# ChalmersPhotonicsLab/QAMpy

Hardware: AMD Instinct MI355X
Metric: equalised MSym/s (2-pol, 2 SPS) (higher is better)
Workload: dtype f32

## Files before the change

qampy_amd/csrc/api.hip:

```cpp
#include "common.h"
#include <stdlib.h>
#include <atomic>
#include <mutex>
#include <vector>
#include <unordered_map>
#include <string.h>

namespace qh {

thread_local hipStream_t g_stream = nullptr;
static thread_local hipStream_t g_streams[4] = {nullptr, nullptr, nullptr, nullptr};
int g_device = -1;
static thread_local std::string g_err;
static std::mutex g_mu;

void set_error(const std::string &s) { g_err = s; }

int hip_fail(hipError_t e, const char *what, const char *file, int line)
{
    g_err = std::string(hipGetErrorString(e)) + " in " + what + " (" + file + ":" + std::to_string(line) + ")";
    (void)hipGetLastError();
    return QH_ERR_HIP;
}

// ... 33 lines not shown
    }
    int n = 0;
    if (hipGetDeviceCount(&n) != hipSuccess || n <= 0) {
        (void)hipGetLastError();
        set_error("no HIP device visible: libqampy_hip needs a gfx950 (MI355X) GPU, there is no CPU fallback");
        return QH_ERR_NODEVICE;
    }
    if (device < 0 || device >= n) { set_error("device index out of range"); return QH_ERR_ARG; }
    hipDeviceProp_t prop;
    QH_HIP(hipGetDeviceProperties(&prop, device));
    if (strncmp(prop.gcnArchName, "gfx950", 6) != 0) {
        set_error(std::string("device is ") + prop.gcnArchName + ", libqampy_hip is built for gfx950 only");
        return QH_ERR_NODEVICE;
    }
    QH_HIP(hipSetDevice(device));
    int prio_least = 0, prio_greatest = 0;
    QH_HIP(hipDeviceGetStreamPriorityRange(&prio_least, &prio_greatest));
    for (int i = 0; i < 4; i++) {
        if (g_streams[i]) { (void)hipStreamDestroy(g_streams[i]); g_streams[i] = nullptr; }
        if (i == 2) {
            const int reserved = reserved_cus();
            const int ncu = prop.multiProcessorCount;
            if (reserved > 0 && reserved < ncu) {
                std::vector<uint32_t> mask((ncu + 31) / 32, 0u);
                for (int c = reserved; c < ncu; c++) mask[c / 32] |= 1u << (c % 32);
                if (hipExtStreamCreateWithCUMask(&g_streams[i], (uint32_t)mask.size(), mask.data()) == hipSuccess) continue;
                (void)hipGetLastError();
                g_streams[i] = nullptr;
            }
        }
        QH_HIP(hipStreamCreateWithPriority(&g_streams[i], hipStreamNonBlocking, i == 2 ? prio_least : prio_greatest));
    }
    g_stream = g_streams[0];
    g_device = device;
    return QH_OK;
}

hipStream_t side_stream() { return g_stream == g_streams[0] ? g_streams[1] : g_streams[0]; }
hipStream_t helper_stream() { return g_streams[3]; }

int ensure_init()
{
    if (g_stream) return QH_OK;
    return init_device(g_device >= 0 ? g_device : 0);
}

thread_local void *g_scratch[SCRATCH_SLOTS] = {nullptr};
thread_local size_t g_scratch_n[SCRATCH_SLOTS] = {0};
thread_local unsigned g_scratch_epoch = 0;
static std::atomic<int> g_form[FORM_COUNT];
struct FormName { const char *key, *env; };
static const FormName FORM_NAMES[FORM_COUNT] = {
    {"trainer", "QAMPY_HIP_TRAINER"}, {"pit_form", "QAMPY_HIP_PIT_FORM"}, {"seg_lanes", "QAMPY_HIP_SEG_LANES"}, {"pit_probe", "QAMPY_HIP_PIT_PROBE"},
    {"bps", "QAMPY_HIP_BPS"}};
static int form_parse(int k, const char *v, int *out)
{
    if (!v || !v[0]) { *out = 0; return 0; }
    switch (k) {
    case FORM_TRAINER: *out = v[0] == 'd' ? 1 : (v[0] == 'l' ? 2 : (v[0] == 'i' ? 3 : (v[0] == 'a' || v[0] == '0' ? 0 : -1))); break;
    case FORM_PIT: *out = v[0] == 's' ? 1 : (v[0] == 'b' ? 2 : (v[0] == 'a' || v[0] == '0' ? 0 : -1)); break;
    case FORM_SEG_LANES: { const int n = atoi(v); *out = (n == 8 || n == 16 || n == 0) ? n : -1; break; }
    case FORM_BPS: *out = v[0] == 't' ? 1 : (v[0] == 'l' ? 2 : (v[0] == 'a' || v[0] == '0' ? 0 : -1)); break;
    default: *out = atoi(v) != 0 ? 1 : 0; break;
    }
    return *out < 0 ? -1 : 0;
}
static const int g_form_env_read = [] {
    for (int k = 0; k < FORM_COUNT; k++) {
        int v = 0;
        if (form_parse(k, getenv(FORM_NAMES[k].env), &v) == 0) g_form[k].store(v);
    }
    return 0;
}();
int form(FormKey k) { return g_form[k].load(std::memory_order_relaxed); }
const char *trainer_force()
{
    switch (form(FORM_TRAINER)) {
    case 1: return "direct";
    case 2: return "lookahead";
    case 3: return "iterative";
    default: return "";
    }
}
static constexpr int POOL_CLASSES = 48, POOL_KEEP = 8;
static constexpr size_t POOL_BYTES = (size_t)24 << 30;
static std::vector<void *> g_pool[POOL_CLASSES];
static size_t g_pool_bytes = 0;
static void pool_release();
static int pool_class(size_t bytes) { int k = 8; while (((size_t)1 << k) < bytes && k < POOL_CLASSES - 1) k++; return k; }
int pool_alloc(size_t bytes, void **p, size_t *cap)
{
    const int k = pool_class(bytes);
    *cap = (size_t)1 << k;
    {
        std::lock_guard<std::mutex> lk(g_mu);
        if (!g_pool[k].empty()) { *p = g_pool[k].back(); g_pool[k].pop_back(); g_pool_bytes -= *cap; return QH_OK; }
    }
    hipError_t e = hipMalloc(p, *cap);
    if (e == hipErrorOutOfMemory) {
        (void)hipGetLastError();
        (void)hipDeviceSynchronize();
        pool_release();
        e = hipMalloc(p, *cap);
    }
    QH_HIP(e);
    return QH_OK;
}
// ... 348 lines not shown
```

qampy_amd/csrc/common.h:

```cpp
#pragma once
#include <hip/hip_runtime.h>
#include <stdint.h>
#include <string>
#include "../../include/qampy_hip.h"

namespace qh {

extern thread_local hipStream_t g_stream;
extern int g_device;
void set_error(const std::string &s);
int hip_fail(hipError_t e, const char *what, const char *file, int line);

#define QH_HIP(call)                                                        \
    do {                                                                    \
        hipError_t _e = (call);                                             \
        if (_e != hipSuccess) return qh::hip_fail(_e, #call, __FILE__, __LINE__); \
    } while (0)

#define QH_REQUIRE(cond, msg)                                   \
    do {                                                        \
        if (!(cond)) { qh::set_error(msg); return QH_ERR_ARG; } \
    } while (0)

#define QH_WAVE_FIRST() __builtin_amdgcn_s_setprio(3)

int ensure_init();
hipStream_t side_stream();
hipStream_t helper_stream();
enum FormKey { FORM_TRAINER = 0, FORM_PIT, FORM_SEG_LANES, FORM_PIT_PROBE, FORM_BPS, FORM_COUNT };
int form(FormKey k);
const char *trainer_force();
double gram_budget_gb();
int pit_timing_mode();
int default_tier();
double default_tier_tol();
constexpr int SCRATCH_SLOTS = 22;
constexpr int SCRATCH_TWOSTAGE = 16;
constexpr int SCRATCH_FOE = 17;
constexpr int SCRATCH_IMPAIR = 18;
constexpr int SCRATCH_PMD = 19;
constexpr int SCRATCH_TXRESP = 20;
constexpr int SCRATCH_SOS = 21;
int scratch(int slot, size_t bytes, void **p);
unsigned scratch_epoch();

int bps_twostage_recover_f32(const void *E, int nm, int64_t L, const void *angles, int A, int B, const void *symbols, int M, int N, int32_t *idx1,
                             int32_t *idx2, void *ph, void *Eout);
int bps_twostage_recover_f64(const void *E, int nm, int64_t L, const void *angles, int A, int B, const void *symbols, int M, int N, int32_t *idx1,
                             int32_t *idx2, void *ph, void *Eout);

int pool_alloc(size_t bytes, void **p, size_t *cap);
void pool_free(void *p, size_t cap);

struct DevBuf {
    void *p = nullptr;
    size_t n = 0, cap = 0;
    ~DevBuf() { if (p) pool_free(p, cap); }
    int alloc(size_t bytes) {
        n = bytes;
        return pool_alloc(bytes ? bytes : 1, &p, &cap);
    }
    int from_host(const void *h, size_t bytes) {
        int rc = alloc(bytes);
        if (rc) return rc;
        if (bytes) QH_HIP(hipMemcpyAsync(p, h, bytes, hipMemcpyHostToDevice, g_stream));
        return QH_OK;
    }
    int to_host(void *h, size_t bytes) const {
        if (bytes) QH_HIP(hipMemcpyAsync(h, p, bytes, hipMemcpyDeviceToHost, g_stream));
        return QH_OK;
    }
};

template <typename R> struct Cx { R re, im; };

template <typename R> struct Cx2T;
template <> struct Cx2T<float> { using type = float2; };
template <> struct Cx2T<double> { using type = double2; };

template <typename R> __device__ __forceinline__ Cx<R> ldg(const Cx<R> *p)
{
    using V = typename Cx2T<R>::type;
// ... 82 lines not shown
```

qampy_amd/csrc/train_pit.h:

```cpp
#pragma once
#include <atomic>
#include <chrono>
#include <vector>
#include "train_impl.h"
#include "train_seg.h"

namespace qh {

typedef qh_pit_report PitCtrl;

constexpr double PIT_CONTRACT = 0.2;
constexpr int PIT_PROBE = 128;
constexpr int PIT_SEEDWIN = 512;
constexpr int PIT_MAXSEG = 65536;

__host__ __device__ inline int pit_symmetry(int method)
{
    switch (method) {
    case QH_M_CMA: case QH_M_SGNCMA: case QH_M_RDE: return 0;
    case QH_M_CMA2: return 2;
    default: return 4;
    }
}

// ... 1220 lines not shown
            const int k = k0 + 4 * i;
            if (k < np) {
                Zf a = abuf[i];
                abuf[i] = lda(k + 4 * PF);
                if (MODE == 0) a.y = -a.y;
                const Zf b = bp[(size_t)k * PIT_MBP];
                rr = __builtin_amdgcn_mfma_f32_16x16x4f32(a.x, b.x, rr, 0, 0, 0);
                ii = __builtin_amdgcn_mfma_f32_16x16x4f32(a.y, b.y, ii, 0, 0, 0);
                im = __builtin_amdgcn_mfma_f32_16x16x4f32(a.x, b.y, im, 0, 0, 0);
                im = __builtin_amdgcn_mfma_f32_16x16x4f32(a.y, b.x, im, 0, 0, 0);
            }
        }
    }
    const int cl = lane & 15;
    if (MODE == 0) {
        const int col = col0 + cl;
#pragma unroll
        for (int q = 0; q < 4; q++) {
            const int m = 16 * wave + 4 * (lane >> 4) + q;
            if (m < n && col < ncol) Out[(size_t)m * ncol + col] = Zf{rr[q] - ii[q], im[q]};
        }
    } else {
#pragma unroll
        for (int q = 0; q < 4; q++) {
            const int m = 16 * wave + 4 * (lane >> 4) + q;
            Ct[cl * (PIT_EIGMAX + 1) + m] = Zf{rr[q] - ii[q], im[q]};
        }
        __syncthreads();
        for (int cb = 0; cb < PIT_MC; cb += NCW * nw) {
#pragma unroll
            for (int q = 0; q < NCW; q++) {
                const int cc = cb + wave + nw * q, col = col0 + cc;
                if (cc < PIT_MC && col < ncol) {
                    const int s = col / fz.nsel, j = col - s * fz.nsel;
                    const size_t base = (size_t)s * wset + (size_t)fz.modes_dev[j] * n;
                    const double qr = pre ? th[q][0] : fz.theta[2 * (size_t)col], qi = pre ? th[q][1] : fz.theta[2 * (size_t)col + 1];
#pragma unroll
                    for (int h = 0; h < 2; h++) {
                        const int m = lane + 64 * h;
                        if (m < n) {
                            const Cx<R> x = pre ? xv[q][h] : fz.X[base + m];
                            const Zf d = Ct[cc * (PIT_EIGMAX + 1) + m];
                            const Cx<R> w{(R)(qr * x.re - qi * x.im + fz.damp * d.x), (R)(qr * x.im + qi * x.re + fz.damp * d.y)};
                            fz.X[base + m] = w;
                            fz.Y[base + m] = w;
                        }
                    }
                }
            }
        }
    }
}

static __global__ void __launch_bounds__(256) pit_bound_kernel(const Zf *Xe, const Zf *Ye, const Zf *Yprev, const double *lam, int n, int S, int nsel, int sym,
                                                              const PitCtrl *c, double *dfc, double *pw, double *gph, float4 *ualpha = nullptr)
{
    QH_WAVE_FIRST();
    if (c->done) return;
    const int lane = threadIdx.x & 63, bi = blockIdx.x * 4 + (threadIdx.x >> 6);
    const int nb = (S - 1) * nsel, ncol = S * nsel;
    if (bi >= nb + nsel) return;
    const bool result_probe = bi >= nb;
    const int j = result_probe ? bi - nb : bi % nsel;
    const int sb = result_probe ? S - 1 : bi / nsel;
    const Zf *pa = result_probe ? (c->passes == 0 ? Xe + (size_t)(S - 1) * nsel + j : Yprev + j) : Xe + (size_t)(sb + 1) * nsel + j;
    const size_t sa = (result_probe && c->passes != 0) ? (size_t)nsel : (size_t)ncol;
    const Zf *pb = Ye + (size_t)sb * nsel + j;
    Zf av[(PIT_EIGMAX + 63) / 64], bv[(PIT_EIGMAX + 63) / 64];
    float lv[(PIT_EIGMAX + 63) / 64];
    double A = 0, B = 0, Cr = 0, Ci = 0;
#pragma unroll
    for (int q = 0; q < (PIT_EIGMAX + 63) / 64; q++) {
        const int k = lane + 64 * q;
        av[q] = Zf{0.f, 0.f}; bv[q] = Zf{0.f, 0.f}; lv[q] = 0.f;
        if (k < n) {
            av[q] = pa[(size_t)k * sa]; bv[q] = pb[(size_t)k * ncol];
            const float l = (float)lam[k];
            lv[q] = l > 0.f ? l : 0.f;
        }
        A += (double)lv[q] * ((double)av[q].x * av[q].x + (double)av[q].y * av[q].y);
        B += (double)lv[q] * ((double)bv[q].x * bv[q].x + (double)bv[q].y * bv[q].y);
        Cr += (double)lv[q] * ((double)bv[q].x * av[q].x + (double)bv[q].y * av[q].y);
        Ci += (double)lv[q] * ((double)bv[q].y * av[q].x - (double)bv[q].x * av[q].y);
    }
    for (int o = 32; o > 0; o >>= 1) { A += __shfl_xor(A, o); B += __shfl_xor(B, o); Cr += __shfl_xor(Cr, o); Ci += __shfl_xor(Ci, o); }
    double gr = 1, gi = 0;
    if (sym == 0) {
        const double pr = sqrt(Cr * Cr + Ci * Ci);
        if (pr > 0) { gr = Cr / pr; gi = Ci / pr; }
    } else if (sym == 4 || sym == 2 || sym == 1) {
        if (sym == 4 && fabs(Ci) > fabs(Cr)) { gr = 0; gi = Ci >= 0 ? 1 : -1; }
        else if (sym == 1) gr = 1;
        else gr = Cr >= 0 ? 1 : -1;
    } else {
        const double step = 6.283185307179586 / sym;
        const double kk = rint(atan2(Ci, Cr) / step) * step;
        gr = cos(kk); gi = sin(kk);
    }
    double d2 = 0;
    const float grf = (float)gr, gif = (float)gi;
#pragma unroll
    for (int q = 0; q < (PIT_EIGMAX + 63) / 64; q++) {
        const float dr = bv[q].x - (grf * av[q].x - gif * av[q].y), di = bv[q].y - (grf * av[q].y + gif * av[q].x);
        d2 += (double)lv[q] * ((double)dr * dr + (double)di * di);
    }
    for (int o = 32; o > 0; o >>= 1) d2 += __shfl_xor(d2, o);
    if (ualpha && !result_probe) {
        float nn = 0.f, ar = 0.f, ai = 0.f;
#pragma unroll
        for (int q = 0; q < (PIT_EIGMAX + 63) / 64; q++) {
            const float dr = bv[q].x - (grf * av[q].x - gif * av[q].y), di = bv[q].y - (grf * av[q].y + gif * av[q].x);
            const float ur = lv[q] * bv[q].x, ui = lv[q] * bv[q].y;
            nn += ur * ur + ui * ui;
            ar += ur * dr + ui * di;
            ai += ur * di - ui * dr;
        }
        for (int o = 32; o > 0; o >>= 1) { nn += __shfl_xor(nn, o); ar += __shfl_xor(ar, o); ai += __shfl_xor(ai, o); }
        const float inv = nn > 0.f ? rsqrtf(nn) : 0.f;
        if (lane == 0) ualpha[bi] = float4{ar * inv, ai * inv, inv, 0.f};
    }
    if (lane == 0) {
        if (!result_probe) { gph[2 * (size_t)bi] = gr; gph[2 * (size_t)bi + 1] = gi; pw[bi] = B; }
        dfc[bi] = (A == A && B == B) ? sqrt(d2 / (B > 1e-300 ? B : 1e-300)) : 1e30;
    }
}

constexpr int PIT_RT = 1024;
template <typename R>
__global__ void __launch_bounds__(PIT_RT) pit_recur_eig_kernel(Zf *Xe, const Zf *Ye, Zf *D, const double *theta, const double *lam, int nsel, int S, int64_t T, const R *mu,
                                                               double beta, const PitCtrl *c, const float *Msum = nullptr, float damp = 1.f,
                                                               const float4 *ualpha = nullptr, const float2 *uq = nullptr)
{
    QH_WAVE_FIRST();
    if (c->done) return;
    __shared__ float4 aff[2 * PIT_RT];
    const int k = blockIdx.x, j = blockIdx.y;
    const int ncol = S * nsel;
    Zf *row = D + (size_t)k * ncol + j, *xr = Xe + (size_t)k * ncol + j;
    const Zf *yr = Ye + (size_t)k * ncol + j;
    double a = (double)*mu * c->gain * (double)T * lam[k];
    if (a < 0) a = 0;
    const float coef = c->corr_on ? (float)exp(-a * (1 + beta * a)) : 0.f;
    const float gl = (float)(c->gain * lam[k] > 0 ? c->gain * lam[k] : 0.0), betaf = (float)beta;
    const bool corr = c->corr_on != 0;
    auto cf = [&](int s) -> float {
        if (!Msum) return coef;
        const float as = gl * Msum[(size_t)s * nsel + j];
        return corr ? __expf(-as * (1.f + betaf * as)) : 0.f;
    };
    const int len = (S + PIT_RT - 1) / PIT_RT;
    const int s0 = threadIdx.x * len, s1 = s0 + len < S ? s0 + len : S;
    auto th = [&](int s) { return Zf{(float)theta[2 * ((size_t)s * nsel + j)], (float)theta[2 * ((size_t)s * nsel + j) + 1]}; };
    auto scan_op = [](float4 e, float4 l) { return float4{l.x * e.x, l.x * e.y + l.y, l.x * e.z + l.z, 0.f}; };
    if (len <= 4) {
        Zf y[4], x[4], t[5], r[4];
        t[0] = s0 > 0 && s0 < S ? th(s0 - 1) : Zf{1.f, 0.f};
#pragma unroll
        for (int q = 0; q < 4; q++) {
            const int s = s0 + q;
            const bool ok = s < s1;
            y[q] = (ok && s > 0) ? yr[(size_t)(s - 1) * nsel] : Zf{0.f, 0.f};
            x[q] = ok ? xr[(size_t)s * nsel] : Zf{0.f, 0.f};
            t[q + 1] = ok ? th(s) : Zf{1.f, 0.f};
        }
        Zf run{0.f, 0.f};
        float cq[4], clen = 1.f;
        float4 ua[4];
        float2 qq[4];
        const float lk = (float)(lam[k] > 0 ? lam[k] : 0.0);
#pragma unroll
        for (int q = 0; q < 4; q++) {
            const int s = s0 + q;
            cq[q] = (s < s1 && s > 0) ? cf(s - 1) : (s < s1 ? 0.f : 1.f);
            ua[q] = (ualpha && s < s1 && s > 0) ? ualpha[(size_t)(s - 1) * nsel + j] : float4{0.f, 0.f, 0.f, 0.f};
            qq[q] = (uq && s < s1 && s > 0) ? uq[(size_t)s * nsel + j] : float2{0.f, 0.f};
        }
        Zf uk[4];
#pragma unroll
        for (int q = 0; q < 4; q++) {
            const int s = s0 + q;
// ... 153 lines not shown
    const int s0 = threadIdx.x * len, s1 = s0 + len < n ? s0 + len : n;
    auto seg_map = [&](int s, double &A, double &B) {
        const double rho = (double)rS[s], d = (double)rE[s] - rho;
        double kappa = 0;
        if (newton && pass >= 2) {
            const double rp = (double)rPrev[s], dp = (double)dPrev[s];
            if (fabs(rho - rp) > 1e-6 * rho && fabs(d) > 1e-30) kappa = -((d - dp) / d) / ((rho - rp) / rho);
            kappa = kappa == kappa ? (kappa < 0 ? 0 : (kappa > 4 ? 4 : kappa)) : 0;
        }
        A = 1.0 - kappa * d / rho;
        B = d * (1.0 + kappa);
    };
    double Ac = 1, Bc = 0;
    for (int s = s0; s < s1; s++) { double A, B; seg_map(s, A, B); Bc = A * Bc + B; Ac = A * Ac; }
    auto comp = [](double2 e, double2 l) { return double2{l.x * e.x, l.x * e.y + l.y}; };
    const double2 pre = block_scan_excl<double2, decltype(comp), 1024>(double2{Ac, Bc}, comp, double2{1.0, 0.0}, buf);
    double run = pre.x * (double)rS[0] + pre.y;
    float worst = 0.f;
    for (int s = s0; s < s1; s++) {
        double A, B;
        seg_map(s, A, B);
        const float old = (float)rS[s];
        rPrev[s] = old; dPrev[s] = (float)((double)rE[s] - (double)old);
        if (s > 0) {
            const float nw = pass == 0 ? (float)run : old + relax * ((float)run - old);
            const float rel = fabsf(nw - old) / (fabsf(old) > 1e-30f ? fabsf(old) : 1e-30f);
            worst = (rel > worst || !(rel == rel)) ? (rel == rel ? rel : 3.0e38f) : worst;
            rS[s] = (R)nw;
            eS[s] = eE[s - 1];
        }
        run = A * run + B;
    }
    for (int o = 32; o > 0; o >>= 1) { const float w2 = __shfl_xor(worst, o); worst = worst > w2 ? worst : w2; }
    if ((threadIdx.x & 63) == 0) red[threadIdx.x >> 6] = worst;
    __syncthreads();
    if (threadIdx.x == 0) { float m = 0.f; for (int w = 0; w < 16; w++) m = m > red[w] ? m : red[w]; chg[0] = m; }
}
template <typename R> __global__ void pit_adapt_finish_kernel(R *mu, const R *rE, int n) { *mu = (R)1 / rE[n - 1]; }

struct PitInit { void *z[3]; unsigned zn[3]; void *cd[2]; const void *cs[2]; unsigned cn[2]; int64_t *modes_dev; int64_t modes[16]; int nsel; };
static __global__ void __launch_bounds__(256) pit_init_kernel(PitInit a)
{
    QH_WAVE_FIRST();
    const unsigned t = blockIdx.x * 256 + threadIdx.x, nt = gridDim.x * 256;
#pragma unroll
    for (int r = 0; r < 3; r++)
        if (a.z[r]) for (unsigned i = t; i < a.zn[r] / 4; i += nt) reinterpret_cast<uint32_t *>(a.z[r])[i] = 0u;
#pragma unroll
    for (int r = 0; r < 2; r++)
        if (a.cd[r]) for (unsigned i = t; i < a.cn[r] / 8; i += nt) reinterpret_cast<uint64_t *>(a.cd[r])[i] = reinterpret_cast<const uint64_t *>(a.cs[r])[i];
    if ((int)t < a.nsel) a.modes_dev[t] = a.modes[t];
}
constexpr int PIT_GT_THREADS = 1024;
template <typename R>
__global__ void __launch_bounds__(PIT_GT_THREADS) pit_gauge_kernel(const double *gph, int S, int nsel, PitCtrl *c, double *theta, const double *pw, int nb, int method, const Cx<R> *sy0,
                                                                   int want_corr, const PitModel *model = nullptr, const float4 *ualpha = nullptr, float2 *uq = nullptr,
                                                                   const R *mu = nullptr, int64_t T = 0, const float *Msum = nullptr)
{
    QH_WAVE_FIRST();
    if (c->done) return;
    constexpr int NT = PIT_GT_THREADS;
    __shared__ double redp[NT / 64];
    __shared__ double2 gbuf[NT / 64];
    __shared__ float4 abuf[NT / 64];
    if (gridDim.x > 1 && blockIdx.x == 1 && !(model && uq)) return;
    if (model && uq && (gridDim.x == 1 || blockIdx.x == 1)) {
        const bool corr = c->passes == 0 ? true : c->corr_on != 0;
        const int len = (S + NT - 1) / NT;
        const int s0 = threadIdx.x * len, s1 = s0 + len < S ? s0 + len : S;
        const float muT = mu ? (float)((double)*mu * (double)T) : 0.f;
        auto op = [](float4 e, float4 l) { return float4{l.x * e.x, l.x * e.y + l.y, l.z * e.z, l.z * e.w + l.w}; };
        for (int j = 0; j < nsel; j++) {
            const PitModel m = model[j];
            const bool on = corr && m.ok;
            auto cf = [&](int s, float &c1, float &c2) {
                const float t = Msum ? Msum[(size_t)s * nsel + j] : muT;
                c1 = on ? __expf(-fmaxf(m.k1, 0.f) * t) : 0.f; c2 = on ? __expf(-fmaxf(m.k2, 0.f) * t) : 0.f;
            };
            float4 loc{1.f, 0.f, 1.f, 0.f};
            for (int s = s0; s < s1; s++) {
                float b1 = 0.f, b2 = 0.f, c1 = 0.f, c2 = 0.f;
                if (s > 0) { const float4 al = ualpha[(size_t)(s - 1) * nsel + j]; b1 = m.q11 * al.x + m.q21 * al.y; b2 = m.q12 * al.x + m.q22 * al.y; cf(s - 1, c1, c2); }
                loc = op(loc, float4{c1, b1, c2, b2});
            }
            const float4 pre = block_scan_excl<float4, decltype(op), NT>(loc, op, float4{1.f, 0.f, 1.f, 0.f}, abuf);
            float r1 = pre.y, r2 = pre.w;
            for (int s = s0; s < s1; s++) {
                float b1 = 0.f, b2 = 0.f, c1 = 0.f, c2 = 0.f;
                if (s > 0) { const float4 al = ualpha[(size_t)(s - 1) * nsel + j]; b1 = m.q11 * al.x + m.q21 * al.y; b2 = m.q12 * al.x + m.q22 * al.y; cf(s - 1, c1, c2); }
                r1 = c1 * r1 + b1; r2 = c2 * r2 + b2;
                uq[(size_t)s * nsel + j] = float2{m.q11 * r1 + m.q12 * r2, m.q21 * r1 + m.q22 * r2};
            }
        }
        if (gridDim.x > 1) return;
    }
    if (c->passes == 0) {
        double ps = 0;
        for (int i = threadIdx.x; i < nb; i += NT) ps += pw[i];
        for (int o = 32; o > 0; o >>= 1) ps += __shfl_xor(ps, o);
        if ((threadIdx.x & 63) == 0) redp[threadIdx.x >> 6] = ps;
        __syncthreads();
        if (threadIdx.x == 0) {
            double tot = 0;
            for (int w = 0; w < NT / 64; w++) tot += redp[w];
            const double Py = tot / (nb > 0 ? nb : 1);
            double g = pit_gain<R>(method, Py, sy0[0]);
            if (model) {
                double gs = 0; int ng = 0;
                for (int j = 0; j < nsel; j++) if (model[j].ok) { gs += (double)model[j].g; ng++; }
                if (ng == nsel && gs > 0) g = gs / ng;
            }
            c->out_power = Py; c->gain = g;
            c->corr_on = (want_corr && g > 0 && g == g) ? 1 : 0;
        }
        __syncthreads();
    }
    const int len = (S + NT - 1) / NT;
    const int s0 = threadIdx.x * len, s1 = s0 + len < S ? s0 + len : S;
    auto cm = [](double2 x, double2 y) { return double2{x.x * y.x - x.y * y.y, x.x * y.y + x.y * y.x}; };
    const double2 *g2 = reinterpret_cast<const double2 *>(gph);
    double2 *th2 = reinterpret_cast<double2 *>(theta);
    if (len <= 4 && nsel <= 2) {
        double2 g[2][4];
#pragma unroll
        for (int j = 0; j < 2; j++)
#pragma unroll
            for (int q = 0; q < 4; q++) {
                const int s = s0 + q;
                g[j][q] = (j < nsel && s < s1 && s > 0) ? g2[(size_t)(s - 1) * nsel + j] : double2{1.0, 0.0};
            }
#pragma unroll
        for (int j = 0; j < 2; j++) {
            if (j >= nsel) break;
            const double2 prod = cm(cm(g[j][0], g[j][1]), cm(g[j][2], g[j][3]));
            double2 run = block_scan_excl<double2, decltype(cm), NT>(prod, cm, double2{1.0, 0.0}, gbuf);
#pragma unroll
            for (int q = 0; q < 4; q++) {
                const int s = s0 + q;
                run = cm(run, g[j][q]);
                if (s < s1) {
                    const double r = rsqrt(run.x * run.x + run.y * run.y);
                    th2[(size_t)s * nsel + j] = double2{run.x * r, run.y * r};
                }
            }
        }
        return;
    }
    for (int j = 0; j < nsel; j++) {
        double2 prod{1.0, 0.0};
        for (int s = s0; s < s1; s++)
            if (s > 0) prod = cm(prod, g2[(size_t)(s - 1) * nsel + j]);
        double2 run = block_scan_excl<double2, decltype(cm), NT>(prod, cm, double2{1.0, 0.0}, gbuf);
        for (int s = s0; s < s1; s++) {
            if (s > 0) run = cm(run, g2[(size_t)(s - 1) * nsel + j]);
            const double r = rsqrt(run.x * run.x + run.y * run.y);
            th2[(size_t)s * nsel + j] = double2{run.x * r, run.y * r};
        }
    }
}
template <typename R>
__global__ void __launch_bounds__(256) pit_devest_kernel(const Zf *D, const double *lam, int n, int ncol, const PitCtrl *c, float *devmax, unsigned *ticket, PitDecideArgs<R> da)
{
    QH_WAVE_FIRST();
    if (c->done) return;
    __shared__ float part[2][4][64], red[64], reds[64], redt[64], redm[64];
    const int cl = threadIdx.x & 63, kg = threadIdx.x >> 6;
    const int col = blockIdx.x * 64 + cl;
    float acc = 0.f, tap = 0.f;
    if (col < ncol) {
#pragma unroll 8
        for (int k = kg; k < n; k += 4) {
            const Zf v = D[(size_t)k * ncol + col];
            const float l = (float)lam[k], m2 = v.x * v.x + v.y * v.y;
            acc += (l > 0.f ? l : 0.f) * m2;
            tap += m2;
        }
    }
    part[0][kg][cl] = acc; part[1][kg][cl] = tap;
    __syncthreads();
    if (kg == 0) {
        acc = (part[0][0][cl] + part[0][1][cl]) + (part[0][2][cl] + part[0][3][cl]);
        tap = (part[1][0][cl] + part[1][1][cl]) + (part[1][2][cl] + part[1][3][cl]);
        red[cl] = (acc == acc) ? acc : 3.0e38f;
        reds[cl] = (acc == acc) ? acc : 3.0e38f;
        redt[cl] = (tap == tap) ? tap : 3.0e38f;
        redm[cl] = (tap == tap) ? tap : 3.0e38f;
    }
    __syncthreads();
    for (int s = 32; s > 0; s >>= 1) {
        if (threadIdx.x < s) {
            red[threadIdx.x] = red[threadIdx.x] > red[threadIdx.x + s] ? red[threadIdx.x] : red[threadIdx.x + s];
            reds[threadIdx.x] += reds[threadIdx.x + s];
            redt[threadIdx.x] += redt[threadIdx.x + s];
            redm[threadIdx.x] = redm[threadIdx.x] > redm[threadIdx.x + s] ? redm[threadIdx.x] : redm[threadIdx.x + s];
        }
        __syncthreads();
    }
    if (threadIdx.x == 0) {
        devmax[4 * blockIdx.x] = red[0]; devmax[4 * blockIdx.x + 1] = reds[0]; devmax[4 * blockIdx.x + 2] = redt[0]; devmax[4 * blockIdx.x + 3] = redm[0];
    }
    __shared__ int last;
    if (threadIdx.x == 0) {
        __threadfence();
        const unsigned t = atomicAdd(ticket, 1u);
        last = t == gridDim.x - 1;
        if (last) { *ticket = 0; __threadfence(); }
    }
    __syncthreads();
    if (!last) return;
    pit_decide_body<R>(da);
}
// ... 332 lines not shown
        if (t > seg_want) seg_want = t;
    }
    if (S == 0 && adaptive) S = (int)((TrSyms - head) / seg_want < PIT_MAXSEG ? (TrSyms - head) / seg_want : PIT_MAXSEG);
    if (S == 0) {
        R mu_h = (R)o.mu_hint;
        if (!(o.mu_hint > 0)) {
            QH_HIP(hipMemcpyAsync(&mu_h, mu_dev, sizeof(R), hipMemcpyDeviceToHost, g_stream));
            QH_HIP(hipStreamSynchronize(g_stream));
        }
        S = pit_auto_segments(TrSyms, (double)mu_h, nsel, o.acquire);
    }
    PitPlan pl = pit_plan(o, TrSyms, head, S, adaptive, o.acquire ? o.acq_chunk : 0);
    const PitSeg &sg = pl.sg;
    if (zero_err) QH_HIP(hipMemsetAsync(err, 0, (size_t)nmodes * TrSyms * Niter * sizeof(Cx<R>), g_stream));
    const int64_t npow = L < 4096 ? L : 4096;
    hipLaunchKernelGGL((pit_setup_kernel<R>), dim3(1), dim3(256), 0, g_stream, (const Cx<R> *)E, nmodes, L, npow, ntot, (const R *)mu_dev, pl.gear, pl.bound, tol, sg, ctrl, mu_acq);
    QH_HIP(hipGetLastError());
    if (TrSyms == 0 || Niter == 0) return QH_OK;
    if (sg.S < 2) {
        const double zero = 0;
        QH_HIP(hipMemcpyAsync(&ctrl->defect[0], &zero, sizeof(double), hipMemcpyHostToDevice, g_stream));
        return exact_form(ctrl, adaptive ? 1 : 0, 0, gram, 1);
    }

    TrainerForm f;
    if ((rc = trainer_form<R>(f, FORM_PASSES, method, adaptive, nmodes, ntaps, os, sg.len, (int64_t)sg.S * nsel, symbols, nsy, modes, nsel))) return rc;
    if (adaptive && !f.seg) return exact_form(ctrl, 1, 0, nullptr, 0);
    const bool decision = method == QH_M_SBD || method == QH_M_MDDMA || method == QH_M_DD;
    const bool seg_form = f.seg, use_bi = f.use_bi, block_form = f.block, pair_tab = f.pair_tab;
    const bool split = o.exchange != nullptr;
    const int own_first = split ? o.seg_first : 0, own_count = split ? o.seg_count : sg.S;
    const bool xchg_async = split && o.exchange_on_stream != 0;
    if (split) {
        QH_REQUIRE(seg_form, "train_equaliser: a capture split over processes needs the throughput form of the passes (>= 512 chains, supported tap layout)");
        QH_REQUIRE(own_first >= 0 && own_count >= 0 && own_first + own_count <= sg.S, "train_equaliser: owned segments outside the segment grid");
        QH_REQUIRE(Niter == 1, "train_equaliser: a capture split over processes is trained in one sweep");
    }

    const size_t wset = (size_t)nmodes * ntot;
    const size_t wbytes = wset * sizeof(Cx<R>);
    void *wbuf = nullptr;
    const size_t nsj = (size_t)sg.S * nsel;
    const size_t bytes_w = ((2 * (size_t)sg.S + 2) * wbytes + 63) / 64 * 64;
    if ((rc = scratch(2, bytes_w + 10 * nsj * sizeof(double) + (size_t)nsel * sizeof(int64_t) + 320 + nsj * 16 + 4 * ((nsj + 63) / 64) * sizeof(float) + 64, &wbuf))) return rc;
    Cx<R> *X = (Cx<R> *)wbuf, *Y = X + (size_t)sg.S * wset, *w_start = Y + (size_t)sg.S * wset, *w_call = w_start + wset;
    double *z = (double *)((char *)wbuf + bytes_w), *rot = z + 2 * nsj, *dfc = rot + 2 * nsj, *pw = dfc + nsj, *gph = pw + nsj, *theta = gph + 2 * nsj;
    int64_t *modes_dev = (int64_t *)(theta + 2 * nsj);
    double *uw_phi = (double *)(modes_dev + ((nsel + 7) / 8 * 8));
    int *uw_jump = (int *)(uw_phi + (size_t)sg.S * nsel);
    float *devmax = (float *)(uw_jump + (size_t)sg.S * nsel);
    const int ndev = (int)((nsj + 63) / 64);
    unsigned *ticket = (unsigned *)(devmax + 4 * (size_t)ndev);
    PitInit init{};
    init.z[0] = ticket; init.zn[0] = sizeof(unsigned);
    R *ad_rS = nullptr, *ad_rE = nullptr;
    Cx<R> *ad_eS = nullptr, *ad_eE = nullptr, *ad_errh = nullptr;
    float *ad_M = nullptr, *ad_chg = nullptr, *ad_rP = nullptr, *ad_dP = nullptr;
    if (!adaptive && head > 0) {
        void *ab = nullptr;
        if ((rc = scratch(13, (size_t)nmodes * head * sizeof(Cx<R>) + 64, &ab))) return rc;
        ad_errh = (Cx<R> *)ab;
    }
    if (adaptive) {
        void *ab = nullptr;
        const size_t nS = ((size_t)sg.S + 15) / 16 * 16;
        if ((rc = scratch(13, nS * (2 * sizeof(R) + 2 * sizeof(Cx<R>) + 3 * sizeof(float)) + 64 + (size_t)nmodes * head * sizeof(Cx<R>), &ab))) return rc;
        ad_eS = (Cx<R> *)ab; ad_eE = ad_eS + nS; ad_errh = ad_eE + nS;
        ad_rS = (R *)(ad_errh + (size_t)nmodes * head); ad_rE = ad_rS + nS;
        ad_M = (float *)(ad_rE + nS); ad_rP = ad_M + nS; ad_dP = ad_rP + nS; ad_chg = ad_dP + nS;
    }
    init.modes_dev = modes_dev; init.nsel = nsel;
    for (int j = 0; j < 16; j++) init.modes[j] = j < nsel ? modes[j] : 0;
    const bool prepared = o.prepared != nullptr && o.acquire && !adaptive && head == 0 && Niter >= 1;
    const bool need_mu = adaptive || !(o.mu_hint > 0), need_acq = o.acquire && !(o.acq_chunk > 0) && !prepared;
    R mu_acq_h = 0;
    if (need_acq) QH_HIP(hipMemcpyAsync(&mu_acq_h, mu_acq, sizeof(R), hipMemcpyDeviceToHost, g_stream));
    R mu_host = need_mu ? (R)1 : (R)o.mu_hint;
    if (need_mu) QH_HIP(hipMemcpyAsync(&mu_host, mu_dev, sizeof(R), hipMemcpyDeviceToHost, g_stream));
    if (need_mu || need_acq) QH_HIP(hipStreamSynchronize(g_stream));
    if (!adaptive && !(mu_host != 0))
        return exact_form(ctrl, 0, 0, gram, 0);
    if (o.acquire && !(o.acq_chunk > 0)) pl.acquisition(o, TrSyms, pit_acq_chunk(mu_acq_h));

    const int64_t amax = pl.amax;
    void *G = const_cast<void *>(gram);
    if (prepared) QH_REQUIRE(seg_form && o.acq_chunk > 0, "train_equaliser: a prepared acquisition belongs to throughput-form passes with acq_chunk given (qh_pit_prepare_*_dev said so)");
    if (block_form && !G && (!seg_form || amax > 0) && !prepared) {
        const int64_t n = seg_form ? pl.ngram : TrSyms;
        rc = pair_tab ? gram_build<R>(E, nmodes, L, os, ntaps, n, &G) : gram_cur_build<R>(E, nmodes, L, os, ntaps, n, &G);
        if (rc) return rc;
    }
    const int64_t g_per_step = pair_tab ? LA_B : GRAM_TRI / 2 / LA_B;

    const int ncol = sg.S * nsel;
    const double *lam = nullptr;
    const Zf *Vb = nullptr;
    Zf *Dz[2] = {nullptr, nullptr};
    Zf *Xe = nullptr, *Ye = nullptr, *Yprev = nullptr;
    if (want_corr) {
        void *cb = nullptr;
        if ((rc = scratch(10, pit_basis_bytes(ntot) + 4 * (size_t)ntot * ncol * sizeof(Zf) + (size_t)ntot * nsel * sizeof(Zf) + 256, &cb))) return rc;
        void *basis = o.basis ? o.basis : cb;
        if (!o.basis && (rc = pit_basis<R>(E, nmodes, L, os, ntaps, TrSyms, basis))) return rc;
        lam = (const double *)basis; Vb = (const Zf *)((const char *)basis + (size_t)ntot * sizeof(double));
        Dz[0] = (Zf *)((char *)cb + (pit_basis_bytes(ntot) + 63) / 64 * 64); Dz[1] = Dz[0] + (size_t)ntot * ncol;
        Xe = Dz[1] + (size_t)ntot * ncol; Ye = Xe + (size_t)ntot * ncol; Yprev = Ye + (size_t)ntot * ncol;
    }
    const bool eig = want_corr && sizeof(R) == 4 && form(FORM_PIT_PROBE) == 0;
    const bool tables_ok = method == QH_M_CMA || method == QH_M_SGNCMA || method == QH_M_MCMA || method == QH_M_RDE || method == QH_M_MRDE ||
                           (decision && (use_bi || seg_form));
    const bool ssb = eig && tables_ok && method != QH_M_CMA2;
    PitModel *model = nullptr;
    float4 *ualpha = nullptr;
    float2 *uqv = nullptr;
    PitModelArgs<R> ma;
    hipEvent_t model_event = nullptr;
    if (ssb) {
        void *mb = nullptr;
        const size_t pw_ = 2 * PIT_EIGMAX + 8;
        const size_t b_part = (size_t)PIT_MODB * 4 * nsel * pw_ * sizeof(float), b_u = ((size_t)nsel * ntot * sizeof(Cx<R>) + 63) / 64 * 64;
        const size_t b_ua = ((size_t)ncol * sizeof(float4) + 63) / 64 * 64, b_uq = ((size_t)ncol * sizeof(float2) + 63) / 64 * 64;
        if ((rc = scratch(14, b_part + b_u + b_ua + b_uq + 16 * sizeof(PitModel) + 128, &mb))) return rc;
        ma.part = (float *)mb; ma.u = (Cx<R> *)((char *)mb + b_part);
        ualpha = (float4 *)((char *)mb + b_part + b_u); uqv = (float2 *)((char *)ualpha + b_ua);
        model = (PitModel *)((char *)uqv + b_uq); ma.model = model; ma.ticket = (unsigned *)(model + 16);
        init.z[1] = ma.ticket; init.zn[1] = sizeof(unsigned);
        init.z[2] = ualpha; init.zn[2] = (unsigned)(b_ua + b_uq);
        ma.E = (const Cx<R> *)E; ma.wx = (const Cx<R> *)wx; ma.L = L; ma.TrSyms = TrSyms; ma.nmodes = nmodes; ma.ntaps = ntaps; ma.os = os; ma.nsel = nsel; ma.method = method;
        if (decision) { ma.symbols = (const Cx<R> *)f.dd_table; ma.nsy = 2 * f.dd_npart + 1; ma.sy_pitch = 2 * BI_DD_MAXLEV; ma.tables = 1; }
        else { ma.symbols = (const Cx<R> *)symbols; ma.nsy = nsy; ma.sy_pitch = nsy; ma.tables = (method == QH_M_RDE || method == QH_M_MRDE) ? 1 : 0; }
        for (int j = 0; j < 16; j++) ma.modes[j] = j < nsel ? modes[j] : 0;
        if (o.corr_beta < 0) beta = 0.0;
    }
    const size_t glds = ((size_t)PIT_EIGMAX * PIT_EIGMAX + (size_t)PIT_EIGMAX * PIT_GT) * sizeof(Zf);
    static std::atomic<bool> gemm_attr{false};
    if (want_corr && !gemm_attr.load(std::memory_order_acquire)) {
        QH_HIP(hipFuncSetAttribute((const void *)pit_cgemm_kernel<R, true>, hipFuncAttributeMaxDynamicSharedMemorySize, 160 * 1024 - 256));
        QH_HIP(hipFuncSetAttribute((const void *)pit_cgemm_kernel<R, false>, hipFuncAttributeMaxDynamicSharedMemorySize, 160 * 1024 - 256));
        QH_HIP(hipFuncSetAttribute((const void *)pit_basis_mfma_kernel<R, 0>, hipFuncAttributeMaxDynamicSharedMemorySize, 128 * 1024));
        QH_HIP(hipFuncSetAttribute((const void *)pit_basis_mfma_kernel<R, 1>, hipFuncAttributeMaxDynamicSharedMemorySize, 128 * 1024));
        gemm_attr.store(true, std::memory_order_release);
    }

    LaArgs<R> la = la_args<R>(E, L, nmodes, ntaps, os, modes, nsel, method, symbols, nsy, mu_dev, err, TrSyms * Niter);
    la.G = (const GramPair<R> *)G; la.gpair = pair_tab ? 1 : 0; la.wx_cs = (int64_t)wset;
    la.dd_general = f.dd_general;
    f.alphabet(la);
    const TrainArgs<R> ta = train_args<R>(E, L, nmodes, ntaps, os, TrSyms, Niter, modes, nsel, method, symbols, nsy, mu_dev, err);

    PitTiming &tm = pit_timing();
    tm.npass = 0; tm.acq_ms = 0;
    bool acq_timed = false;
    PitEvents &ev = pit_events();
    QH_REQUIRE(ev.ok, "train_equaliser: no pinned memory for the pass flags");
    const bool redo_ok = o.exact_redo_off == 0;
    bool fell_back = false;
    if (redo_ok && !adaptive) { init.cd[0] = w_call; init.cs[0] = wx; init.cn[0] = (unsigned)wbytes; }
    if (o.acquire && Niter > 0) { init.cd[1] = w_start; init.cs[1] = wx; init.cn[1] = (unsigned)wbytes; }
    hipLaunchKernelGGL(pit_init_kernel, dim3(32), dim3(256), 0, g_stream, init);
    QH_HIP(hipGetLastError());
    for (int it = 0; it < Niter; it++) {
// ... 86 lines not shown
                g_stream = keep;
            }
            if (timed(p)) QH_HIP(hipEventRecord(ev.t0[p], g_stream));
            if (seg_form) {
                SegArgs<R> sa{};
                sa.E = (const Cx<R> *)E; sa.wx = Y; sa.symbols = la.symbols; sa.err = (Cx<R> *)err; sa.mu = mu_dev;
                sa.L = L; sa.TrSyms = TrSyms; sa.nsy = la.nsy; sa.sy_pitch = la.sy_pitch; sa.err_pitch = TrSyms * Niter; sa.err_off = (int64_t)it * TrSyms;
                sa.nmodes = nmodes; sa.ntaps = ntaps; sa.os = os; sa.nsel = nsel; sa.S = sg.S;
                sa.seg_len = sg.len; sa.seg_extra = sg.extra; sa.seg_tail = sg.tail; sa.seg_begin = sg.begin;
                sa.r_in = ad_rS; sa.r_out = ad_rE; sa.e_in = ad_eS; sa.e_out = ad_eE; sa.mu_sum = (R *)ad_M; sa.adapt_first = sg.begin > 0 ? 1 : 0;
                for (int j = 0; j < 16; j++) sa.modes[j] = j < nsel ? modes[j] : 0;
                sa.skip = &ctrl->done;
                sa.q_first = own_first * nsel; sa.q_count = split ? own_count * nsel : 0;
                pit_last_launch().form = 1;
                if (!split || own_count > 0) { int r = launch_seg<R>(sa, method, adaptive); if (r) return r; }
                if (adaptive) hipLaunchKernelGGL((pit_adapt_scan_kernel<R>), dim3(1), dim3(1024), 0, g_stream, ad_rS, (const R *)ad_rE, ad_eS, (const Cx<R> *)ad_eE, sg.S, ad_chg, (const PitCtrl *)ctrl, ad_relax, ad_rP, ad_dP, ad_newton);
            } else if (block_form) {
                LaArgs<R> ls = la;
                ls.TrSyms = sg.len; ls.nch = sg.S; ls.wx = Y; ls.err_off = (int64_t)it * TrSyms; ls.seg = 1; ls.seg_extra = sg.extra; ls.seg_tail = sg.tail;
                ls.skip = &ctrl->done;
                pit_last_launch() = PitLaunch{use_bi ? 2 : 3, 0, 0, 0, 0, 0};
                if (sg.begin > 0) {
                    ls.E = (const Cx<R> *)E + sg.begin * os; ls.L = L - sg.begin * os; ls.err_off += sg.begin;
                    ls.G = (const GramPair<R> *)G + sg.begin * g_per_step;
                }
                { int r = use_bi ? launch_bi<R>(ls) : launch_la<R>(ls); if (r) return r; }
            } else {
                TrainArgs<R> ts = ta;
                ts.wx = Y; ts.nseg = sg.S; ts.seg_begin = sg.begin; ts.seg_len = sg.len; ts.seg_extra = sg.extra; ts.seg_tail = sg.tail; ts.seg_iter = it; ts.skip = &ctrl->done;
                pit_last_launch() = PitLaunch{4, 0, 0, 0, 0, 0};
                { int r = launch_any<R>(ts); if (r) return r; }
            }
            if (timed(p)) QH_HIP(hipEventRecord(ev.t1[p], g_stream));
            if (split) {
                if (own_first > 0) QH_HIP(hipMemsetAsync(Y, 0, (size_t)own_first * wbytes, g_stream));
                if (own_first + own_count < sg.S)
                    QH_HIP(hipMemsetAsync(Y + (size_t)(own_first + own_count) * wset, 0, (size_t)(sg.S - own_first - own_count) * wbytes, g_stream));
                if (!xchg_async) QH_HIP(hipStreamSynchronize(g_stream));
                if (o.exchange(o.exchange_user, Y, (size_t)sg.S * wbytes) != 0) { set_error("train_equaliser: the exchange callback failed"); return QH_ERR_ARG; }
            }
            const int nbnd = (int)((sg.S - 1) * nsel);
            if (eig) {
                if (o.basis && pit_basis_sync().pending) {
                    QH_HIP(hipStreamWaitEvent(g_stream, pit_basis_sync().out, 0));
                    pit_basis_sync().pending = false;
                }
                auto forward2 = [&](const Cx<R> *src, Zf *dst, const Cx<R> *src2, Zf *dst2) {
                    PitFuse<R> f2 = fz;
                    f2.T2 = src2; f2.Out2 = reinterpret_cast<float2 *>(dst2);
                    hipLaunchKernelGGL((pit_basis_mfma_kernel<R, 0>), dim3(2 * ((ncol + PIT_MC - 1) / PIT_MC)), dim3(pit_mfma_threads(ntot)), pit_mfma_lds(ntot), g_stream, Vb, src, (const Zf *)nullptr, dst, ntot, ncol, (const PitCtrl *)ctrl, f2);
                };
                if (p == 0 && model_event) QH_HIP(hipStreamWaitEvent(g_stream, model_event, 0));
                forward2((const Cx<R> *)X, Xe, (const Cx<R> *)Y, Ye);
                hipLaunchKernelGGL(pit_bound_kernel, dim3((nbnd + nsel + 3) / 4), dim3(256), 0, g_stream, (const Zf *)Xe, (const Zf *)Ye, (const Zf *)Yprev, lam, ntot, sg.S, nsel, sym,
                                   (const PitCtrl *)ctrl, dfc, pw, gph, ualpha);
                hipLaunchKernelGGL((pit_gauge_kernel<R>), dim3(ssb ? 2 : 1), dim3(PIT_GT_THREADS), 0, g_stream, (const double *)gph, sg.S, nsel, ctrl, theta, (const double *)pw,
                                   nbnd, method, (const Cx<R> *)symbols + (size_t)modes[0] * nsy, 1, (const PitModel *)model, (const float4 *)ualpha, uqv,
                                   (const R *)mu_dev, sg.len, (const float *)ad_M);
                hipLaunchKernelGGL((pit_recur_eig_kernel<R>), dim3(ntot, nsel), dim3(PIT_RT), 0, g_stream, Xe, (const Zf *)Ye, Dz[1], (const double *)theta, lam, nsel, sg.S, sg.len,
                                   (const R *)mu_dev, beta, (const PitCtrl *)ctrl, (const float *)ad_M, (adaptive && p >= 1) ? ad_damp : 1.f,
                                   (const float4 *)ualpha, (const float2 *)uqv);
                hipLaunchKernelGGL((pit_devest_kernel<R>), dim3(ndev), dim3(256), 0, g_stream, (const Zf *)Dz[1], lam, ntot, ncol, (const PitCtrl *)ctrl, devmax, ticket,
                                   decide_args(p, (const float *)devmax, (const float2 *)Ye, (float2 *)Yprev, ntot, ncol, 1));
            } else {
            const size_t dlds = (2 * (size_t)ntot + (size_t)nmodes * os * pit_phase_pitch(ntaps, os, PIT_PROBE)) * sizeof(Cx<R>);
            QH_REQUIRE(dlds <= 60 * 1024, "train_equaliser: boundary probe does not fit the LDS for this filter shape");
            hipLaunchKernelGGL((pit_defect_kernel<R>), dim3(sg.S, nsel), dim3(PIT_PROBE), dlds, g_stream, (const Cx<R> *)E, nmodes, L, os,
                               ntaps, sg, TrSyms, (const int64_t *)modes_dev, (const Cx<R> *)X, (const Cx<R> *)Y, sym, (const PitCtrl *)ctrl, dfc, pw, gph, (const Cx<R> *)wx);
            hipLaunchKernelGGL((pit_gauge_kernel<R>), dim3(1), dim3(PIT_GT_THREADS), 0, g_stream, (const double *)gph, sg.S, nsel, ctrl, theta, (const double *)pw,
                               nbnd, method, (const Cx<R> *)symbols + (size_t)modes[0] * nsy, want_corr ? 1 : 0);
            if (want_corr) {
                if (o.basis && pit_basis_sync().pending) {
                    QH_HIP(hipStreamWaitEvent(g_stream, pit_basis_sync().out, 0));
                    pit_basis_sync().pending = false;
                }
                hipLaunchKernelGGL((pit_cgemm_kernel<R, true>), dim3((ncol + PIT_GT - 1) / PIT_GT), dim3(256), glds, g_stream, Vb, (const Zf *)nullptr, Dz[1], ntot, ncol, (const PitCtrl *)ctrl, fz);
                hipLaunchKernelGGL((pit_recur_kernel<R>), dim3(ntot, nsel), dim3(256), 0, g_stream, Dz[1], lam, nsel, sg.S, sg.len, (const R *)mu_dev, beta, (const PitCtrl *)ctrl);
                hipLaunchKernelGGL((pit_devest_kernel<R>), dim3(ndev), dim3(256), 0, g_stream, (const Zf *)Dz[1], lam, ntot, ncol, (const PitCtrl *)ctrl, devmax, ticket,
                                   decide_args(p, (const float *)devmax, (const float2 *)nullptr, (float2 *)nullptr, 0, 0, 1));
            } else
                hipLaunchKernelGGL((pit_decide_kernel<R>), dim3(1), dim3(256), 0, g_stream, decide_args(p, (const float *)nullptr, (const float2 *)nullptr, (float2 *)nullptr, 0, 0, 0));
            }
            QH_HIP(hipGetLastError());
            return QH_OK;
        };
        if ((rc = enqueue_pass(0))) return rc;
        if (it == 0 && o.on_pass0) {
            hipStream_t keep = g_stream;
            o.on_pass0(o.on_pass0_user);
            g_stream = keep;
        }
        bool ahead = false;
        bool certified = false;
        for (int p = 0; p < npass; p++) {
            double contr = PIT_CONTRACT;
            if (p >= 2 && ev.hview[2 * (p - 2) + 1] > 0) {
                contr = (double)ev.hview[2 * (p - 1) + 1] / (double)ev.hview[2 * (p - 2) + 1];
                contr = contr < 0.1 ? 0.1 : (contr > 0.9 ? 0.9 : contr);
            }
            const bool expect_last = p > 0 && contr * (double)ev.hview[2 * (p - 1) + 1] < tol;
            ahead = false;
            if (p + 1 < npass && !expect_last && (!split || xchg_async)) { if ((rc = enqueue_pass(p + 1))) return rc; ahead = true; }
            {
                volatile float *hv = (volatile float *)ev.hview;
                unsigned spins = 0;
                auto t_last = std::chrono::steady_clock::now();
                while (hv[2 * p] < 0.f) {
                    if ((++spins & 255u) != 0) continue;
                    const auto now = std::chrono::steady_clock::now();
                    if (now - t_last < std::chrono::milliseconds(20)) continue;
                    t_last = now;
// ... 130 lines not shown
```

Baseline: 1199.

## Fuse PIT boundary probe and gauge kernels via last-block ticket handover

Merges pit_bound_kernel and pit_gauge_kernel into one launch for the eigen path. Blocks take a ticket with an atomic counter after finishing their boundary work, and the last block to arrive runs the gauge body. This removes one kernel launch and the gap between the two kernels inside each training pass. In exchange the gauge step, including the ssb uq scan that used to run in its own second block, now runs serially in a single block. Blocks are also 1024 threads instead of 256, and correctness depends on the fences and on the ticket counter being reset.

```diff
diff --git a/qampy_amd/csrc/api.hip b/qampy_amd/csrc/api.hip
--- a/qampy_amd/csrc/api.hip
+++ b/qampy_amd/csrc/api.hip
@@ -109,7 +109,7 @@
 struct FormName { const char *key, *env; };
 static const FormName FORM_NAMES[FORM_COUNT] = {
     {"trainer", "QAMPY_HIP_TRAINER"}, {"pit_form", "QAMPY_HIP_PIT_FORM"}, {"seg_lanes", "QAMPY_HIP_SEG_LANES"}, {"pit_probe", "QAMPY_HIP_PIT_PROBE"},
-    {"bps", "QAMPY_HIP_BPS"}};
+    {"bps", "QAMPY_HIP_BPS"}, {"pit_six", "QAMPY_HIP_PIT_SIX"}};
 static int form_parse(int k, const char *v, int *out)
 {
     if (!v || !v[0]) { *out = 0; return 0; }
diff --git a/qampy_amd/csrc/common.h b/qampy_amd/csrc/common.h
--- a/qampy_amd/csrc/common.h
+++ b/qampy_amd/csrc/common.h
@@ -27,7 +27,7 @@
 int ensure_init();
 hipStream_t side_stream();
 hipStream_t helper_stream();
-enum FormKey { FORM_TRAINER = 0, FORM_PIT, FORM_SEG_LANES, FORM_PIT_PROBE, FORM_BPS, FORM_COUNT };
+enum FormKey { FORM_TRAINER = 0, FORM_PIT, FORM_SEG_LANES, FORM_PIT_PROBE, FORM_BPS, FORM_PIT_SIX, FORM_COUNT };
 int form(FormKey k);
 const char *trainer_force();
 double gram_budget_gb();
diff --git a/qampy_amd/csrc/train_pit.h b/qampy_amd/csrc/train_pit.h
--- a/qampy_amd/csrc/train_pit.h
+++ b/qampy_amd/csrc/train_pit.h
@@ -1296,12 +1296,9 @@
     }
 }
 
-static __global__ void __launch_bounds__(256) pit_bound_kernel(const Zf *Xe, const Zf *Ye, const Zf *Yprev, const double *lam, int n, int S, int nsel, int sym,
-                                                              const PitCtrl *c, double *dfc, double *pw, double *gph, float4 *ualpha = nullptr)
-{
-    QH_WAVE_FIRST();
-    if (c->done) return;
-    const int lane = threadIdx.x & 63, bi = blockIdx.x * 4 + (threadIdx.x >> 6);
+static __device__ __forceinline__ void pit_bound_body(const Zf *Xe, const Zf *Ye, const Zf *Yprev, const double *lam, int n, int S, int nsel, int sym,
+                                                      const PitCtrl *c, double *dfc, double *pw, double *gph, float4 *ualpha, int bi, int lane)
+{
     const int nb = (S - 1) * nsel, ncol = S * nsel;
     if (bi >= nb + nsel) return;
     const bool result_probe = bi >= nb;
@@ -1368,8 +1365,43 @@
         dfc[bi] = (A == A && B == B) ? sqrt(d2 / (B > 1e-300 ? B : 1e-300)) : 1e30;
     }
 }
+static __global__ void __launch_bounds__(256) pit_bound_kernel(const Zf *Xe, const Zf *Ye, const Zf *Yprev, const double *lam, int n, int S, int nsel, int sym,
+                                                              const PitCtrl *c, double *dfc, double *pw, double *gph, float4 *ualpha = nullptr)
+{
+    QH_WAVE_FIRST();
+    if (c->done) return;
+    pit_bound_body(Xe, Ye, Yprev, lam, n, S, nsel, sym, c, dfc, pw, gph, ualpha, blockIdx.x * 4 + (threadIdx.x >> 6), threadIdx.x & 63);
+}
 
 constexpr int PIT_RT = 1024;
+template <int NT, typename Sink>
+__device__ __forceinline__ void pit_gauge_uq_mode(int j, int S, int nsel, bool corr, const PitModel *model, const float4 *ualpha, float muT, const float *Msum,
+                                                  float4 *abuf, Sink sink)
+{
+    const int len = (S + NT - 1) / NT;
+    const int s0 = threadIdx.x * len, s1 = s0 + len < S ? s0 + len : S;
+    auto op = [](float4 e, float4 l) { return float4{l.x * e.x, l.x * e.y + l.y, l.z * e.z, l.z * e.w + l.w}; };
+    const PitModel m = model[j];
+    const bool on = corr && m.ok;
+    auto cf = [&](int s, float &c1, float &c2) {
+        const float t = Msum ? Msum[(size_t)s * nsel + j] : muT;
+        c1 = on ? __expf(-fmaxf(m.k1, 0.f) * t) : 0.f; c2 = on ? __expf(-fmaxf(m.k2, 0.f) * t) : 0.f;
+    };
+    float4 loc{1.f, 0.f, 1.f, 0.f};
+    for (int s = s0; s < s1; s++) {
+        float b1 = 0.f, b2 = 0.f, c1 = 0.f, c2 = 0.f;
+        if (s > 0) { const float4 al = ualpha[(size_t)(s - 1) * nsel + j]; b1 = m.q11 * al.x + m.q21 * al.y; b2 = m.q12 * al.x + m.q22 * al.y; cf(s - 1, c1, c2); }
+        loc = op(loc, float4{c1, b1, c2, b2});
+    }
+    const float4 pre = block_scan_excl<float4, decltype(op), NT>(loc, op, float4{1.f, 0.f, 1.f, 0.f}, abuf);
+    float r1 = pre.y, r2 = pre.w;
+    for (int s = s0; s < s1; s++) {
+        float b1 = 0.f, b2 = 0.f, c1 = 0.f, c2 = 0.f;
+        if (s > 0) { const float4 al = ualpha[(size_t)(s - 1) * nsel + j]; b1 = m.q11 * al.x + m.q21 * al.y; b2 = m.q12 * al.x + m.q22 * al.y; cf(s - 1, c1, c2); }
+        r1 = c1 * r1 + b1; r2 = c2 * r2 + b2;
+        sink(s, float2{m.q11 * r1 + m.q12 * r2, m.q21 * r1 + m.q22 * r2});
+    }
+}
 template <typename R>
 __global__ void __launch_bounds__(PIT_RT) pit_recur_eig_kernel(Zf *Xe, const Zf *Ye, Zf *D, const double *theta, const double *lam, int nsel, int S, int64_t T, const R *mu,
                                                                double beta, const PitCtrl *c, const float *Msum = nullptr, float damp = 1.f,
@@ -1629,47 +1661,20 @@
     if ((int)t < a.nsel) a.modes_dev[t] = a.modes[t];
 }
 constexpr int PIT_GT_THREADS = 1024;
-template <typename R>
-__global__ void __launch_bounds__(PIT_GT_THREADS) pit_gauge_kernel(const double *gph, int S, int nsel, PitCtrl *c, double *theta, const double *pw, int nb, int method, const Cx<R> *sy0,
-                                                                   int want_corr, const PitModel *model = nullptr, const float4 *ualpha = nullptr, float2 *uq = nullptr,
-                                                                   const R *mu = nullptr, int64_t T = 0, const float *Msum = nullptr)
-{
-    QH_WAVE_FIRST();
-    if (c->done) return;
-    constexpr int NT = PIT_GT_THREADS;
+template <typename R, int NT>
+__device__ __forceinline__ void pit_gauge_body(int nblk, int blk, const double *gph, int S, int nsel, PitCtrl *c, double *theta, const double *pw, int nb, int method,
+                                               const Cx<R> *sy0, int want_corr, const PitModel *model, const float4 *ualpha, float2 *uq, const R *mu, int64_t T, const float *Msum)
+{
     __shared__ double redp[NT / 64];
     __shared__ double2 gbuf[NT / 64];
     __shared__ float4 abuf[NT / 64];
-    if (gridDim.x > 1 && blockIdx.x == 1 && !(model && uq)) return;
-    if (model && uq && (gridDim.x == 1 || blockIdx.x == 1)) {
+    if (nblk > 1 && blk == 1 && !(model && uq)) return;
+    if (model && uq && (nblk == 1 || blk == 1)) {
         const bool corr = c->passes == 0 ? true : c->corr_on != 0;
-        const int len = (S + NT - 1) / NT;
-        const int s0 = threadIdx.x * len, s1 = s0 + len < S ? s0 + len : S;
         const float muT = mu ? (float)((double)*mu * (double)T) : 0.f;
-        auto op = [](float4 e, float4 l) { return float4{l.x * e.x, l.x * e.y + l.y, l.z * e.z, l.z * e.w + l.w}; };
-        for (int j = 0; j < nsel; j++) {
-            const PitModel m = model[j];
-            const bool on = corr && m.ok;
-            auto cf = [&](int s, float &c1, float &c2) {
-                const float t = Msum ? Msum[(size_t)s * nsel + j] : muT;
-                c1 = on ? __expf(-fmaxf(m.k1, 0.f) * t) : 0.f; c2 = on ? __expf(-fmaxf(m.k2, 0.f) * t) : 0.f;
-            };
-            float4 loc{1.f, 0.f, 1.f, 0.f};
-            for (int s = s0; s < s1; s++) {
-                float b1 = 0.f, b2 = 0.f, c1 = 0.f, c2 = 0.f;
-                if (s > 0) { const float4 al = ualpha[(size_t)(s - 1) * nsel + j]; b1 = m.q11 * al.x + m.q21 * al.y; b2 = m.q12 * al.x + m.q22 * al.y; cf(s - 1, c1, c2); }
-                loc = op(loc, float4{c1, b1, c2, b2});
-            }
-            const float4 pre = block_scan_excl<float4, decltype(op), NT>(loc, op, float4{1.f, 0.f, 1.f, 0.f}, abuf);
-            float r1 = pre.y, r2 = pre.w;
-            for (int s = s0; s < s1; s++) {
-                float b1 = 0.f, b2 = 0.f, c1 = 0.f, c2 = 0.f;
-                if (s > 0) { const float4 al = ualpha[(size_t)(s - 1) * nsel + j]; b1 = m.q11 * al.x + m.q21 * al.y; b2 = m.q12 * al.x + m.q22 * al.y; cf(s - 1, c1, c2); }
-                r1 = c1 * r1 + b1; r2 = c2 * r2 + b2;
-                uq[(size_t)s * nsel + j] = float2{m.q11 * r1 + m.q12 * r2, m.q21 * r1 + m.q22 * r2};
-            }
-        }
-        if (gridDim.x > 1) return;
+        for (int j = 0; j < nsel; j++)
+            pit_gauge_uq_mode<NT>(j, S, nsel, corr, model, ualpha, muT, Msum, abuf, [&](int s, float2 q) { uq[(size_t)s * nsel + j] = q; });
+        if (nblk > 1) return;
     }
     if (c->passes == 0) {
         double ps = 0;
@@ -1734,6 +1739,38 @@
             th2[(size_t)s * nsel + j] = double2{run.x * r, run.y * r};
         }
     }
+}
+template <typename R>
+__global__ void __launch_bounds__(PIT_GT_THREADS) pit_gauge_kernel(const double *gph, int S, int nsel, PitCtrl *c, double *theta, const double *pw, int nb, int method, const Cx<R> *sy0,
+                                                                   int want_corr, const PitModel *model = nullptr, const float4 *ualpha = nullptr, float2 *uq = nullptr,
+                                                                   const R *mu = nullptr, int64_t T = 0, const float *Msum = nullptr)
+{
+    QH_WAVE_FIRST();
+    if (c->done) return;
+    pit_gauge_body<R, PIT_GT_THREADS>((int)gridDim.x, (int)blockIdx.x, gph, S, nsel, c, theta, pw, nb, method, sy0, want_corr, model, ualpha, uq, mu, T, Msum);
+}
+template <typename R>
+__global__ void __launch_bounds__(PIT_GT_THREADS) pit_bound_gauge_kernel(const Zf *Xe, const Zf *Ye, const Zf *Yprev, const double *lam, int n, int S, int nsel, int sym, PitCtrl *c,
+                                                                         double *dfc, double *pw, double *gph, float4 *ualpha, unsigned *ticket, double *theta, int method,
+                                                                         const Cx<R> *sy0, int want_corr, const PitModel *model, float2 *uq, const R *mu, int64_t T, const float *Msum)
+{
+    QH_WAVE_FIRST();
+    if (c->done) return;
+    const int lane = threadIdx.x & 63;
+    pit_bound_body(Xe, Ye, Yprev, lam, n, S, nsel, sym, c, dfc, pw, gph, ualpha, blockIdx.x * (PIT_GT_THREADS / 64) + (threadIdx.x >> 6), lane);
+    __shared__ int last;
+    if (lane == 0) __threadfence();
+    __syncthreads();
+    if (threadIdx.x == 0) {
+        const unsigned t = atomicAdd(ticket, 1u);
+        last = t == gridDim.x - 1;
+        if (last) { *ticket = 0; __threadfence(); }
+    }
+    __syncthreads();
+    if (!last) return;
+    __threadfence();
+    if (c->done) return;
+    pit_gauge_body<R, PIT_GT_THREADS>(1, 0, gph, S, nsel, c, theta, pw, (S - 1) * nsel, method, sy0, want_corr, model, (const float4 *)ualpha, uq, mu, T, Msum);
 }
 template <typename R>
 __global__ void __launch_bounds__(256) pit_devest_kernel(const Zf *D, const double *lam, int n, int ncol, const PitCtrl *c, float *devmax, unsigned *ticket, PitDecideArgs<R> da)
@@ -2172,7 +2209,7 @@
     const int ndev = (int)((nsj + 63) / 64);
     unsigned *ticket = (unsigned *)(devmax + 4 * (size_t)ndev);
     PitInit init{};
-    init.z[0] = ticket; init.zn[0] = sizeof(unsigned);
+    init.z[0] = ticket; init.zn[0] = 2 * sizeof(unsigned);
     R *ad_rS = nullptr, *ad_rE = nullptr;
     Cx<R> *ad_eS = nullptr, *ad_eE = nullptr, *ad_errh = nullptr;
     float *ad_M = nullptr, *ad_chg = nullptr, *ad_rP = nullptr, *ad_dP = nullptr;
@@ -2227,6 +2264,7 @@
         Xe = Dz[1] + (size_t)ntot * ncol; Ye = Xe + (size_t)ntot * ncol; Yprev = Ye + (size_t)ntot * ncol;
     }
     const bool eig = want_corr && sizeof(R) == 4 && form(FORM_PIT_PROBE) == 0;
+    const bool handover = eig && form(FORM_PIT_SIX) == 0;
     const bool tables_ok = method == QH_M_CMA || method == QH_M_SGNCMA || method == QH_M_MCMA || method == QH_M_RDE || method == QH_M_MRDE ||
                            (decision && (use_bi || seg_form));
     const bool ssb = eig && tables_ok && method != QH_M_CMA2;
@@ -2419,11 +2457,18 @@
                 };
                 if (p == 0 && model_event) QH_HIP(hipStreamWaitEvent(g_stream, model_event, 0));
                 forward2((const Cx<R> *)X, Xe, (const Cx<R> *)Y, Ye);
+                if (handover)
+                    hipLaunchKernelGGL((pit_bound_gauge_kernel<R>), dim3((nbnd + nsel + PIT_GT_THREADS / 64 - 1) / (PIT_GT_THREADS / 64)), dim3(PIT_GT_THREADS), 0, g_stream,
+                                       (const Zf *)Xe, (const Zf *)Ye, (const Zf *)Yprev, lam, ntot, sg.S, nsel, sym, ctrl, dfc, pw, gph, ualpha, ticket + 1, theta, method,
+                                       (const Cx<R> *)symbols + (size_t)modes[0] * nsy, 1, (const PitModel *)model, uqv, (const R *)mu_dev,
+                                       sg.len, (const float *)ad_M);
+                else {
                 hipLaunchKernelGGL(pit_bound_kernel, dim3((nbnd + nsel + 3) / 4), dim3(256), 0, g_stream, (const Zf *)Xe, (const Zf *)Ye, (const Zf *)Yprev, lam, ntot, sg.S, nsel, sym,
                                    (const PitCtrl *)ctrl, dfc, pw, gph, ualpha);
                 hipLaunchKernelGGL((pit_gauge_kernel<R>), dim3(ssb ? 2 : 1), dim3(PIT_GT_THREADS), 0, g_stream, (const double *)gph, sg.S, nsel, ctrl, theta, (const double *)pw,
                                    nbnd, method, (const Cx<R> *)symbols + (size_t)modes[0] * nsy, 1, (const PitModel *)model, (const float4 *)ualpha, uqv,
                                    (const R *)mu_dev, sg.len, (const float *)ad_M);
+                }
                 hipLaunchKernelGGL((pit_recur_eig_kernel<R>), dim3(ntot, nsel), dim3(PIT_RT), 0, g_stream, Xe, (const Zf *)Ye, Dz[1], (const double *)theta, lam, nsel, sg.S, sg.len,
                                    (const R *)mu_dev, beta, (const PitCtrl *)ctrl, (const float *)ad_M, (adaptive && p >= 1) ? ad_damp : 1.f,
                                    (const float4 *)ualpha, (const float2 *)uqv);
```

After: 997.7. 0.832x the previous value.
